# rendeirolab/stainx

Measured on AMD Instinct MI355X. Metric: megapixels/sec Macenko transform, 64x3x512x512 fp32; max-abs vs torch CPU, higher is better.
Workload: dtype f32; 1 GPU; Macenko reference-mode transform, 64x3x512x512 fp32 per GPU (BASELINE configs[1]); tiles_per_gpu=64, height=512, width=512, input_batches_rotated=2, parallelism=tiles sharded over 1 GPU(s), no collective

## Files before the change

stainx_amd/csrc/macenko.hip:

```cpp
#include "common.hpp"

#include <algorithm>
#include <atomic>
#include <type_traits>
#include <cstdlib>

namespace sx {
namespace macenko {

constexpr int kSample = 4096;
constexpr int kMinCap = 8192;
constexpr int kChunk = 16384;
template <typename T> struct PackOf { static constexpr int n = 16 / (int)sizeof(T); };
constexpr int kSlots = 4;
constexpr int kMoments = 20;
constexpr int kPartial = 10;
constexpr int kShortList = 512;
constexpr int kGroupThreads = 1024;
constexpr int kKeys = kSample / kGroupThreads;
constexpr int kPrefetchHist = 8;
constexpr int kPrefetchCand = 8;
static_assert(kKeys * kGroupThreads == kSample && kPrefetchCand * kGroupThreads <= kMinCap, "per-tile stage geometry");

constexpr float kBeta = 0.15f;
// ... 150 lines not shown

constexpr uint32_t kFusedCapMax = 14336;
static bool fused_size(int64_t pixels) { return pixels >= 16384 && pixels <= 262144 && pixels % 4 == 0; }
static uint32_t fused_cap_for(int64_t pixels) { return (uint32_t)std::min<int64_t>(kFusedCapMax, std::max<int64_t>(2048, (pixels / 4 + 255) / 256 * 256)); }
constexpr uint32_t kDenseCapMax = 24576;
static uint32_t dense_cap_for(int64_t pixels) { return (uint32_t)std::min<int64_t>(kDenseCapMax, std::max<int64_t>(2048, (pixels / 8 + 255) / 256 * 256)); }
static uint32_t record_cap_for(int64_t pixels) { return std::max(fused_cap_for(pixels), dense_cap_for(pixels)); }
static size_t dense_spill_words(int64_t pixels) { return dense_cap_for(pixels) > (uint32_t)kLdsKeys ? (size_t)dense_cap_for(pixels) - kLdsKeys : 0; }
constexpr size_t kFusedSchedBytes = 512, kFusedTileBytes = 64;

enum WorkspaceLevel { kWsBase = 0, kWsFused = 1, kWsTwoPass = 2 };
static bool coded_size(int64_t n_tiles, int64_t pixels) { return pixels % 16 == 0 && n_tiles * pixels >= (1ll << 20); }
static size_t coded_bytes(int64_t n_tiles, int64_t pixels) { return align_up(sizeof(uint32_t) * (size_t)n_tiles, 256) + align_up((size_t)3 * pixels * n_tiles, 256); }
static size_t workspace_bytes(int64_t n_tiles, int64_t pixels, int level = kWsTwoPass) {
    const size_t b = (size_t)blocks_per_tile_for(pixels), n = (size_t)n_tiles;
    size_t total = align_up(sizeof(GroupState) * n, 256);
    total += 2 * align_up(sizeof(double) * kPartial * b * n, 256);
    total += align_up(sizeof(uint32_t) * cand_words(n_tiles, pixels), 256);
    total += align_up(sizeof(uint32_t) * 512 * b * n, 256);
    total += align_up(sizeof(float) * 3 * kSample * n, 256);
    total += align_up(sizeof(PoolState), 256);
    if (level >= kWsFused && two_pass_size(pixels)) {
        total += align_up(kPriorRecordBytes * n, 256);
        total += kFusedSchedBytes;
        total += align_up(kFusedTileBytes * n, 256);
        if (fused_size(pixels)) total += align_up(sizeof(uint4) * kSlots * (size_t)record_cap_for(pixels) * n, 256);
        if (fused_size(pixels)) total += align_up(sizeof(uint32_t) * kSlots * dense_spill_words(pixels) * n, 256);
    }
    if (level >= kWsTwoPass && two_pass_size(pixels)) {
        total += align_up(sizeof(float) * 3 * kSlots * (size_t)cap2_for(pixels) * n, 256);
        total += align_up(sizeof(uint32_t) * kSlots * 256 * n, 256);
        total += align_up(sizeof(uint32_t) * kSlots * key_spill_words(pixels) * n, 256);
    }
    return total;
}

static Workspace carve(void* base, int64_t n_tiles, int64_t pixels, size_t codes_at = 0) {
    Workspace w;
    char* p = static_cast<char*>(base);
    const size_t b = (size_t)blocks_per_tile_for(pixels), n = (size_t)n_tiles;
    w.state = reinterpret_cast<GroupState*>(p);
    p += align_up(sizeof(GroupState) * n, 256);
    w.partial = reinterpret_cast<double*>(p);
    p += align_up(sizeof(double) * kPartial * b * n, 256);
    w.partial_all = reinterpret_cast<double*>(p);
    p += align_up(sizeof(double) * kPartial * b * n, 256);
    w.cand = reinterpret_cast<uint32_t*>(p);
    p += align_up(sizeof(uint32_t) * cand_words(n_tiles, pixels), 256);
    w.block_hist = reinterpret_cast<uint32_t*>(p);
    p += align_up(sizeof(uint32_t) * 512 * b * n, 256);
    w.sample_od = reinterpret_cast<float*>(p);
    p += align_up(sizeof(float) * 3 * kSample * n, 256);
    w.pool = reinterpret_cast<PoolState*>(p);
    p += align_up(sizeof(PoolState), 256);
    {
        char* c = codes_at ? static_cast<char*>(base) + codes_at : p;
        w.code_bad = reinterpret_cast<uint32_t*>(c);
        w.codes = reinterpret_cast<uint8_t*>(c + align_up(sizeof(uint32_t) * n, 256));
    }
    w.prior = reinterpret_cast<PriorRecord*>(p);
    p += align_up(kPriorRecordBytes * n, 256);
    w.fsched = reinterpret_cast<FusedSched*>(p);
    p += kFusedSchedBytes;
    w.ftile = reinterpret_cast<FusedTile*>(p);
    p += align_up(kFusedTileBytes * n, 256);
    w.cand_rec = reinterpret_cast<uint4*>(p);
    if (fused_size(pixels)) p += align_up(sizeof(uint4) * kSlots * (size_t)record_cap_for(pixels) * n, 256);
    w.dense_spill = reinterpret_cast<uint32_t*>(p);
    if (fused_size(pixels)) p += align_up(sizeof(uint32_t) * kSlots * dense_spill_words(pixels) * n, 256);
    w.cand_od = reinterpret_cast<float*>(p);
    p += align_up(sizeof(float) * 3 * kSlots * (size_t)cap2_for(pixels) * n, 256);
    w.seg_count = reinterpret_cast<uint32_t*>(p);
    p += align_up(sizeof(uint32_t) * kSlots * 256 * n, 256);
    w.key_spill = reinterpret_cast<uint32_t*>(p);
    return w;
}

template <typename U> __device__ __forceinline__ void put(U* p, U v) { *p = v; }
template <typename U> __device__ __forceinline__ U get(const U* p) { return *p; }

#ifdef SX_STAMPS
#define SX_STAMP(st, i) do { if (threadIdx.x == 0) (st).stamp[i] = (unsigned long long)wall_clock64(); } while (0)
#define SX_UNIT_STAMP(ws, unit, i) do { if (threadIdx.x == 0) reinterpret_cast<unsigned long long*>((ws).block_hist)[(size_t)(unit) * 8 + (i)] = (unsigned long long)wall_clock64(); } while (0)
#else
#define SX_STAMP(st, i) do { } while (0)
#define SX_UNIT_STAMP(ws, unit, i) do { } while (0)
#endif

template <typename T>
__device__ __forceinline__ float log2_level(float raw) {
    const float t = sizeof(T) == 1 ? raw + 1.0f : fmaf(raw, 255.0f, 1.0f);
    return __log2f(t);
}
template <typename T>
__device__ __forceinline__ float optical_density(float raw) {
    return fmaf(-kLn2, log2_level<T>(raw), kLnIo);
}

template <typename T> struct LevelTables {
    __device__ __forceinline__ void fill() {}
};
template <> struct LevelTables<uint8_t> {
    float od[256], l2[256];
    __device__ __forceinline__ void fill() {
        for (int t = threadIdx.x; t < 256; t += blockDim.x) {
            od[t] = optical_density<uint8_t>((float)t);
            l2[t] = log2_level<uint8_t>((float)t);
        }
        __syncthreads();
    }
};
template <typename F> struct Coded {
    uint8_t v;
    __device__ __forceinline__ operator uint32_t() const { return v; }
};
template <typename T> struct Sem { using type = T; };
template <typename F> struct Sem<Coded<F>> { using type = F; };
template <typename F> __device__ __forceinline__ float code_value(int k) {
    return Elem<F>::load(Elem<F>::store(div255_of_level((float)k)));
}
template <typename F> struct LevelTables<Coded<F>> {
    float od[256], l2[256];
    __device__ __forceinline__ void fill() {
        for (int t = threadIdx.x; t < 256; t += blockDim.x) {
            const float v = code_value<F>(t);
            od[t] = optical_density<F>(v);
            l2[t] = log2_level<F>(v);
        }
        __syncthreads();
    }
};
template <typename F, int kCodeCopies> struct CodeTable {
    static constexpr int copies = kCodeCopies;
    uint2 e[256 * kCodeCopies];
    __device__ __forceinline__ void fill() {
        for (int t = threadIdx.x; t < 256; t += blockDim.x) {
            const float v = code_value<F>(t);
            const uint2 entry = make_uint2(__float_as_uint(v), __float_as_uint(optical_density<F>(v)));
#pragma unroll
            for (int c = 0; c < kCodeCopies; ++c) e[t * kCodeCopies + c] = entry;
        }
        __syncthreads();
    }
};
template <typename T, int V, bool kInter> struct Codable { static constexpr bool value = std::is_same<T, float>::value && V == 4 && !kInter; };

template <typename T> __device__ __forceinline__ float od_of(float v, const LevelTables<T>& tb) {
    if constexpr (sizeof(T) == 1) return tb.od[__float_as_uint(v)]; else return optical_density<T>(v);
}
template <typename T> __device__ __forceinline__ float l2_of(float v, const LevelTables<T>& tb) {
    if constexpr (sizeof(T) == 1) return tb.l2[__float_as_uint(v)]; else return log2_level<T>(v);
}

__device__ __forceinline__ bool od_selected(const float od[3], bool use_all) {
    return use_all || (fminf(od[0], fminf(od[1], od[2])) >= kBeta);
}

__device__ __forceinline__ float diamond_angle(float t1, float t0) {
    const float den = fmaxf(fabsf(t0) + fabsf(t1), 1e-30f);
    const float r = t1 * __builtin_amdgcn_rcpf(den);
    return t0 >= 0.0f ? r : (t1 >= 0.0f ? 2.0f - r : -2.0f - r);
}

__device__ __forceinline__ uint32_t angle_key(const float od[3], const float* __restrict__ v) {
    const float t0 = fmaf(od[2], v[4], fmaf(od[1], v[2], od[0] * v[0]));
    const float t1 = fmaf(od[2], v[5], fmaf(od[1], v[3], od[0] * v[1]));
    return float_key(diamond_angle(t1, t0));
}

__device__ inline float angle_from_key(uint32_t key) {
// ... 3134 lines not shown
```

stainx_amd/csrc/macenko_twopass.hpp:

```cpp
#pragma once

namespace sx {
namespace macenko {

constexpr int kPriorSweeps = 4;
constexpr int kPriorUnitsMax = kGroupThreads / 4 * kPriorSweeps;
constexpr int kQueue2 = 512;
constexpr float kSpecSigmasConc = 5.0f, kSpecThresholdScale = 1.0f;
constexpr float kSpecSigmas = 5.0f;
constexpr float kSpecEffFar = 2.0f, kSpecEffNear = 1.0f;
__device__ __forceinline__ float spec_eff(const Geometry& g) { return g.prior_step_q16 >= (8u << 16) ? g.spec_eff_far : g.spec_eff_near; }
constexpr float kSpecKw = 0.10f, kSpecKx = 1.3e-3f;
constexpr float kSpecRot = 0.30f;
constexpr uint32_t kSpecSlow = 1u, kSpecHazard = 2u;
constexpr int kMaxSegments = 256;

constexpr int kRowBelowA = 0, kRowAboveA = 1, kRowBelowB = 2, kRowAboveB = 3, kRowConc = 4, kRowW = 8;
struct alignas(128) PriorRecord {
    float a0[3], a1[3], an[3];
    float rows[16][4];
    float kw, kx;
    float cmax[4];
    int32_t mode;
    int32_t min_first;
// ... 630 lines not shown
                        }
                        if (__builtin_expect(n_q > (uint32_t)(kQueue2 - kWave), 0)) flush();
                    }
                }
                if constexpr (V > 4) __builtin_amdgcn_sched_barrier(0);
            }
            if (++in_run == kShortRun) {
#pragma unroll
                for (int k = 0; k < kPartial; ++k) {
                    acc[k] += (double)m[k];
                    m[k] = 0.0f;
                }
                in_run = 0;
            }
        }
    };
    if (speculate) sweep(std::true_type{}); else sweep(std::false_type{});
    if (in_run) {
#pragma unroll
        for (int k = 0; k < kPartial; ++k) acc[k] += (double)m[k];
    }

    StatsScratch<TPB>* ss = &sh->stats;
#pragma unroll
    for (int k = 0; k < kPartial; ++k) {
        const double s = wave_total_f64(acc[k]);
        if (lane_id() == kWave - 1) ss->red[wave][k] = s;
    }
    if (speculate) {
        flush();
        if (lane_id() == 0) {
            if constexpr (!kFused) {
                uint32_t* counts = ws.seg_count + ((size_t)tile * kSlots) * g.n_seg + seg;
#pragma unroll
                for (int s = 0; s < kSlots; ++s) put(&counts[(size_t)s * g.n_seg], have[s]);
            }
            if (below_a) atomicAdd(&sh->below[0], below_a);
            if (below_b) atomicAdd(&sh->below[1], below_b);
        }
    }
    __syncthreads();
    if (threadIdx.x < kPartial) {
        double s = 0.0;
#pragma unroll
        for (int w = 0; w < TPB / kWave; ++w) s += ss->red[w][threadIdx.x];
        if constexpr (kFused) st_agent(&ws.partial[item * kPartial + threadIdx.x], s); else put(&ws.partial[item * kPartial + threadIdx.x], s);
    }
    if (speculate && threadIdx.x == kPartial) {
        if (sh->below[0]) atomicAdd(&st.below[0], sh->below[0]);
        if (sh->below[1]) atomicAdd(&st.below[1], sh->below[1]);
    }
    double kept_total = 0.0;
#pragma unroll
    for (int w = 0; w < TPB / kWave; ++w) kept_total += ss->red[w][0];
    if (__builtin_expect(kept_total < 3.0, 0)) {
        if (!tile_has_three_kept_witnesses<T, TPB, kInter>(img, g.pixels)) {
            stats_item_all_pixels<T, V, TPB, kInter>(img, g.pixels, p_begin, p_end, ws.partial_all + item * kPartial, ss);
            if constexpr (kFused) __builtin_amdgcn_fence(__ATOMIC_RELEASE, "agent");
        }
    }
    if constexpr (kFused) {
        drain_stores();
        __syncthreads();
        if (threadIdx.x == 0) __hip_atomic_fetch_add(&ws.ftile[tile].a_done, 1u, __ATOMIC_RELAXED, __HIP_MEMORY_SCOPE_AGENT);
    }
}

template <typename T, int V, bool kInter = false, bool kDense = false>
__global__ __launch_bounds__(kStreamThreads, (Codable<T, V, kInter>::value ? 4 : 1)) void pass_a_kernel(const T* __restrict__ images, Geometry g, Workspace ws) {
    __shared__ PassAScratch<kStreamThreads> sh;
    __shared__ LevelTables<T> tb;
    tb.fill();
    if constexpr (Codable<T, V, kInter>::value) {
        if (g.code_epoch != 0u) {
            __shared__ CodeTable<T, 2> ct;
            ct.fill();
            pass_a_item<T, V, kStreamThreads, kInter, kDense, true>(images, g, ws, blockIdx.x / g.blocks_per_tile, blockIdx.x % g.blocks_per_tile, blockIdx.x, &sh, tb, &ct);
            return;
        }
    }
    pass_a_item<T, V, kStreamThreads, kInter, kDense>(images, g, ws, blockIdx.x / g.blocks_per_tile, blockIdx.x % g.blocks_per_tile, blockIdx.x, &sh, tb);
}

struct alignas(16) SlotScratch {
    TileScratch t;
    uint32_t keys[kLdsKeys];
    float vecs[6], pinv[6], he[6];
    double check[8];
    uint32_t lo, hi, n_list, bin, rank_in_bin, result, range_first, range_last, bin_count;
    int ok, use_all;
    unsigned long long n_sel;
    uint32_t seg_prefix[kMaxSegments + 1], seg_total, seg_overflow, over_n;
    uint32_t dense_n;
    uint32_t own_key;
    int partner_ok;
    uint32_t k_floor, k_ceil, n_under;
};

__device__ __forceinline__ void segment_prefix(SlotScratch* sh, const Geometry& g, const Workspace& ws, int tile, int slot) {
    if (threadIdx.x < kWave) {
        const uint32_t* counts = ws.seg_count + ((size_t)tile * kSlots + slot) * g.n_seg;
        uint32_t c[4], sum = 0, raw = 0;
#pragma unroll
        for (int u = 0; u < 4; ++u) {
            const int k = 4 * (int)threadIdx.x + u;
            const uint32_t v = k < g.n_seg ? get(&counts[k]) : 0u;
            raw += v;
            c[u] = min(v, g.seg_cap);
            sum += c[u];
        }
        const uint32_t incl = wave_scan_u32(sum);
        uint32_t run = incl - sum;
#pragma unroll
        for (int u = 0; u < 4; ++u) {
            const int k = 4 * (int)threadIdx.x + u;
            if (k <= g.n_seg) sh->seg_prefix[k] = run;
            run += c[u];
        }
        const uint32_t total_raw = wave_total_u32(raw);
        if (threadIdx.x == kWave - 1) {
            const uint32_t spilled = get(&ws.state[tile].over_count[slot]);
            sh->seg_prefix[g.n_seg] = incl;
            sh->seg_total = total_raw;
            sh->over_n = min(spilled, g.over_cap);
            sh->seg_overflow = spilled > g.over_cap ? 1u : 0u;
        }
    }
}

template <int kPre> struct CandPrefetch {
    float od[kPre][3];
};
template <int kPre>
__device__ __forceinline__ void prefetch_candidates(CandPrefetch<kPre>& pf, const Geometry& g, const float* __restrict__ c0) {
    const uint32_t team = blockDim.x / (uint32_t)g.n_seg, k = threadIdx.x / team, r = threadIdx.x - k * team;
    const float* src = c0 + (size_t)k * g.seg_cap;
#pragma unroll
    for (int u = 0; u < kPre; ++u) {
        const uint32_t o = r + u * team;
        const bool in = k < (uint32_t)g.n_seg && o < g.seg_cap;
#pragma unroll
        for (int c = 0; c < 3; ++c) pf.od[u][c] = in ? get(&src[(size_t)c * g.cap2 + o]) : 0.0f;
    }
}
template <int kPre, class Fn>
__device__ __forceinline__ void for_each_candidate(const CandPrefetch<kPre>& pf, const SlotScratch* sh, const Geometry& g, const float* __restrict__ c0, Fn fn) {
    const uint32_t team = blockDim.x / (uint32_t)g.n_seg, k = threadIdx.x / team, r = threadIdx.x - k * team;
    const bool mine = k < (uint32_t)g.n_seg;
    const uint32_t first = mine ? sh->seg_prefix[k] : 0u, cnt = mine ? sh->seg_prefix[k + 1] - first : 0u;
    const float* src = c0 + (size_t)k * g.seg_cap;
#pragma unroll
    for (int u = 0; u < kPre; ++u) {
        const uint32_t o = r + u * team;
        if (o < cnt) fn(first + o, pf.od[u]);
    }
    constexpr int kFlight = 4;
    for (uint32_t o = threadIdx.x; o < sh->over_n; o += blockDim.x) {
        const float* p = c0 + (size_t)g.n_seg * g.seg_cap + o;
        const float od[3] = {get(&p[0]), get(&p[g.cap2]), get(&p[2 * (size_t)g.cap2])};
        fn(sh->seg_prefix[g.n_seg] + o, od);
    }
    if (k >= (uint32_t)g.n_seg) return;
    for (uint32_t off = r + kPre * team; off < cnt; off += team * kFlight) {
        float od[kFlight][3];
#pragma unroll
        for (int u = 0; u < kFlight; ++u) {
            const uint32_t o = off + u * team;
#pragma unroll
            for (int c = 0; c < 3; ++c) od[u][c] = o < cnt ? get(&src[(size_t)c * g.cap2 + o]) : 0.0f;
        }
#pragma unroll
        for (int u = 0; u < kFlight; ++u) {
            const uint32_t o = off + u * team;
            if (o < cnt) fn(first + o, od[u]);
        }
    }
}

template <int kPre>
__device__ __forceinline__ void prefetch_candidates_dense(CandPrefetch<kPre>& pf, __amdgpu_buffer_rsrc_t rsrc) {
#pragma unroll
    for (int u = 0; u < kPre; ++u) {
        const sx_u4 rec = __builtin_amdgcn_raw_buffer_load_b128(rsrc, (int)((threadIdx.x + (uint32_t)u * blockDim.x) * 16u), 0, 0);
#pragma unroll
        for (int c = 0; c < 3; ++c) pf.od[u][c] = __uint_as_float(rec[c]);
    }
}
template <int kPre, class Fn>
__device__ __forceinline__ void for_each_candidate_dense(const CandPrefetch<kPre>& pf, uint32_t n, __amdgpu_buffer_rsrc_t rsrc, Fn fn) {
#pragma unroll
    for (int u = 0; u < kPre; ++u) {
        const uint32_t i = threadIdx.x + (uint32_t)u * blockDim.x;
        if (i < n) fn(i, pf.od[u]);
    }
    constexpr int kFlight = 4;
    for (uint32_t i0 = threadIdx.x + (uint32_t)kPre * blockDim.x; i0 < n; i0 += blockDim.x * kFlight) {
        float od[kFlight][3];
#pragma unroll
        for (int u = 0; u < kFlight; ++u) {
            const sx_u4 rec = __builtin_amdgcn_raw_buffer_load_b128(rsrc, (int)((i0 + (uint32_t)u * blockDim.x) * 16u), 0, 0);
#pragma unroll
            for (int c = 0; c < 3; ++c) od[u][c] = __uint_as_float(rec[c]);
        }
#pragma unroll
        for (int u = 0; u < kFlight; ++u) {
            const uint32_t i = i0 + (uint32_t)u * blockDim.x;
            if (i < n) fn(i, od[u]);
        }
    }
}
__device__ __forceinline__ void dense_count(SlotScratch* sh, const Geometry& g, const Workspace& ws, int tile, int slot) {
    if (threadIdx.x == kWave - 1) {
        const uint32_t n_raw = get(&ws.ftile[tile].ncand[slot]);
        sh->seg_total = n_raw;
        sh->dense_n = min(n_raw, g.fused_cap);
        sh->over_n = 0;
        sh->seg_overflow = n_raw > g.fused_cap ? 1u : 0u;
    }
}

__device__ __forceinline__ uint32_t slot_key(const SlotScratch* sh, const uint32_t* __restrict__ spill, uint32_t i) { return i < (uint32_t)kLdsKeys ? sh->keys[i] : get(&spill[i - kLdsKeys]); }

__device__ __forceinline__ void select_prepare(SlotScratch* sh) {
    if (threadIdx.x == 0) {
        sh->lo = 0xFFFFFFFFu;
        sh->hi = 0u;
        sh->n_list = 0;
        sh->result = 0;
        sh->n_under = 0;
    }
    for (int i = threadIdx.x; i < 512; i += blockDim.x) (&sh->t.hist_c[0][0])[i] = 0;
}
__device__ __forceinline__ void publish_range(SlotScratch* sh, uint32_t mn, uint32_t mx) {
    mn = wave_min_u32(mn);
    mx = wave_max_u32(mx);
    if (lane_id() == 0 && mn != 0xFFFFFFFFu) {
        atomicMin(&sh->lo, mn);
        atomicMax(&sh->hi, mx);
    }
}

__device__ uint32_t select_slot_keys(SlotScratch* sh, const uint32_t* __restrict__ spill, uint32_t n, uint32_t rank, bool level0_filled, unsigned long long* dbg = nullptr, uint32_t k_floor = 0u, uint32_t k_ceil = 0xFFFFFFFFu) {
    const uint32_t lane = lane_id();
    const int wave = threadIdx.x / kWave;
    const uint32_t share = ((n + blockDim.x - 1) / blockDim.x) | 1u, i_begin = min(threadIdx.x * share, n), i_end = min(i_begin + share, n);
    const uint32_t lo = max(sh->lo, k_floor), hi = max(min(sh->hi, k_ceil), lo);
    double origin = bin_origin_for(lo), scale = bin_scale_for(lo, hi);
    uint32_t k_first = k_floor, k_last = 0xFFFFFFFFu, want = rank;
    uint32_t picked = 0;
    bool by_bin = false;
    uint32_t* hist = sh->t.hist_c[0];
    for (int level = 0; level < 2; ++level) {
        if (level > 0 || !level0_filled) {
            for (uint32_t i = i_begin; i < i_end; ++i) {
                const uint32_t k = slot_key(sh, spill, i);
                if (k >= k_first && k <= k_last) atomicAdd(&hist[bin_of(k, origin, scale)], 1u);
            }
            __syncthreads();
        }
        if (dbg && threadIdx.x == 0) dbg[level] = (unsigned long long)wall_clock64();
        if (wave == 0) {
            uint32_t b, rb;
            scan_pick32(hist, want, b, rb);
            if (lane == 0) {
                const uint32_t in_bin = hist[b];
                sh->bin = b;
                sh->rank_in_bin = rb;
                sh->bin_count = in_bin;
                if (in_bin > (uint32_t)kShortList || level == 1) {
                    uint32_t first, last;
                    bin_key_range(b, origin, scale, first, last);
                    sh->range_first = max(first, k_first);
                    sh->range_last = min(last, k_last);
                }
            }
        }
        __syncthreads();
        want = sh->rank_in_bin;
        picked = sh->bin;
        const uint32_t in_bin = sh->bin_count;
        if (in_bin <= (uint32_t)kShortList && level == 0) {
            by_bin = true;
            break;
        }
        k_first = sh->range_first;
        k_last = sh->range_last;
        if (level == 1) break;
        if (k_first == k_last) return k_first;
        hist = sh->t.hist_c[1];
        origin = bin_origin_for(k_first);
        scale = bin_scale_for(k_first, k_last);
    }
    if (!by_bin && k_first == k_last) return k_first;
    uint32_t* list = &sh->t.keys[0][0];
    for (uint32_t i = i_begin; i < i_end; ++i) {
        const uint32_t k = slot_key(sh, spill, i);
        if (k >= k_first && k <= k_last && (!by_bin || bin_of(k, origin, scale) == picked)) {
            const uint32_t at = atomicAdd(&sh->n_list, 1u);
            if (at < (uint32_t)(2 * kSample)) list[at] = k;
        }
    }
    __syncthreads();
    if (dbg && threadIdx.x == 0) dbg[2] = (unsigned long long)wall_clock64();
    const uint32_t n_list = sh->n_list;
    if (__builtin_expect(n_list <= (uint32_t)kShortList, 1)) {
        rank_pick(list, n_list, want, threadIdx.x, blockDim.x, &sh->result);
        __syncthreads();
        return sh->result;
    }
    if (n_list <= (uint32_t)(2 * kSample)) return radix_select_stream((unsigned long long)n_list, (unsigned long long)want, [list](unsigned long long i, uint32_t& k) { k = list[i]; return true; }, &sh->t);
    return radix_select_stream((unsigned long long)n, (unsigned long long)rank, [sh, spill, k_floor](unsigned long long i, uint32_t& k) { k = slot_key(sh, spill, (uint32_t)i); return k >= k_floor; }, &sh->t);
}

__device__ inline void frame_coordinates(const PriorRecord* pr, const float x[3], float out[3]) {
    const float f00 = pr->a0[0], f10 = pr->a0[1], f20 = pr->a0[2];
    const float f01 = pr->a1[0], f11 = pr->a1[1], f21 = pr->a1[2];
    const float f02 = pr->an[0], f12 = pr->an[1], f22 = pr->an[2];
    const float c00 = f11 * f22 - f12 * f21, c01 = f12 * f20 - f10 * f22, c02 = f10 * f21 - f11 * f20;
    const float det = f00 * c00 + f01 * c01 + f02 * c02;
    const float inv = det != 0.0f ? __builtin_amdgcn_rcpf(det) : 0.0f;
    const float i00 = c00 * inv, i01 = (f02 * f21 - f01 * f22) * inv, i02 = (f01 * f12 - f02 * f11) * inv;
    const float i10 = c01 * inv, i11 = (f00 * f22 - f02 * f20) * inv, i12 = (f02 * f10 - f00 * f12) * inv;
    const float i20 = c02 * inv, i21 = (f01 * f20 - f00 * f21) * inv, i22 = (f00 * f11 - f01 * f10) * inv;
    out[0] = i00 * x[0] + i01 * x[1] + i02 * x[2];
    out[1] = i10 * x[0] + i11 * x[1] + i12 * x[2];
    out[2] = i20 * x[0] + i21 * x[1] + i22 * x[2];
}

template <typename T>
__device__ void exact_plane(const Geometry& g, const Workspace& ws, int tile, SlotScratch* sh) {
    const int64_t first = (int64_t)tile * g.blocks_per_tile;
    if (threadIdx.x < kPartial) {
        double running = 0.0;
        for (int64_t b0 = 0; b0 < g.blocks_per_tile; b0 += 16) {
            double part[16];
#pragma unroll
            for (int u = 0; u < 16; ++u) part[u] = b0 + u < g.blocks_per_tile ? get(&ws.partial[(first + b0 + u) * kPartial + threadIdx.x]) : 0.0;
#pragma unroll
            for (int u = 0; u < 16; ++u)
                if (b0 + u < g.blocks_per_tile) running += part[u];
        }
        sh->t.mom[threadIdx.x] = running;
    }
    if (threadIdx.x == kPartial) sh->t.mom[kPartial] = (double)g.pixels;
    if (threadIdx.x > kPartial && threadIdx.x < kMoments) sh->t.mom[threadIdx.x] = 0.0;
    __syncthreads();
    if (__builtin_expect(sh->t.mom[0] < 3.0, 0)) {
        __syncthreads();
        if (threadIdx.x < kPartial) {
            double running = 0.0;
            for (int64_t b = 0; b < g.blocks_per_tile; ++b) running += get(&ws.partial_all[(first + b) * kPartial + threadIdx.x]);
            sh->t.mom[kPartial + threadIdx.x] = running;
        }
        __syncthreads();
    }
    if (threadIdx.x < 2) {
        double cov[9];
        bool use_all;
        unsigned long long n_sel;
        float vecs[6];
        plane_from_moments<true>(sh->t.mom, true, cov, vecs, use_all, n_sel);
        if (threadIdx.x == 0) {
#pragma unroll
            for (int i = 0; i < 6; ++i) sh->vecs[i] = vecs[i];
            sh->use_all = use_all ? 1 : 0;
            sh->n_sel = n_sel;
            if ((blockIdx.x & 1) == 0) {
                GroupState& st = ws.state[tile];
#pragma unroll
                for (int i = 0; i < 6; ++i) {
                    put(&st.vecs[i], vecs[i]);
                    put(&st.rec[0].coef[i], vecs[i]);
                }
#pragma unroll
                for (int k = 0; k < kMoments; ++k) put(&st.mom[k], sh->t.mom[k]);
#pragma unroll
                for (int i = 0; i < 9; ++i) put(&st.cov[i], cov[i]);
                put(&st.use_all, use_all ? 1 : 0);
                put(&st.rec[0].use_all, use_all ? 1 : 0);
                put(&st.n_sel, n_sel);
            }
        }
    }
    __syncthreads();
}

__device__ inline bool phi_slot_check(const PriorRecord* pr, const float (&v)[6], int j, double (&check)[8], float rot_limit) {
    float m0[3], m1[3];
    const float v0[3] = {v[0], v[2], v[4]}, v1[3] = {v[1], v[3], v[5]};
    frame_coordinates(pr, v0, m0);
    frame_coordinates(pr, v1, m1);
    const float r00 = m0[0], r01 = m0[1], r10 = m1[0], r11 = m1[1], nu0 = m0[2], nu1 = m1[2];
    const float det = r00 * r11 - r01 * r10;
    const float nu = __builtin_amdgcn_sqrtf(nu0 * nu0 + nu1 * nu1);
    const float stretch = __builtin_amdgcn_sqrtf(r00 * r00 + r01 * r01 + r10 * r10 + r11 * r11);
    const float kw = get(&pr->kw), kx = get(&pr->kx);
    bool good = det > 0.9f && stretch < 1.6f && r00 > 0.8f && r11 > 0.8f && fabsf(r01) + fabsf(r10) < rot_limit && kx >= 1.2e-3f;
    {
        const float a1_min = fminf(pr->a1[0], fminf(pr->a1[1], pr->a1[2]));
        const float a0_max = fmaxf(fabsf(pr->a0[0]), fmaxf(fabsf(pr->a0[1]), fabsf(pr->a0[2])));
        const float an_max = fmaxf(fabsf(pr->an[0]), fmaxf(fabsf(pr->an[1]), fabsf(pr->an[2])));
        if (!(r11 * a1_min > 1.05f * (fabsf(r10) * a0_max + nu * an_max))) good = false;
    }
    const uint32_t open = get(&pr->open);
#pragma unroll
    for (int e = 0; e < 2; ++e) {
        const float* row = pr->rows[2 * j + e];
        float gq[3];
        frame_coordinates(pr, row, gq);
        const float dx = gq[1], dy = -gq[0];
        const float mx = r00 * dx + r01 * dy, my = r10 * dx + r11 * dy;
        const bool is_open = ((open >> (2 * j + e)) & 1u) != 0;
        check[e] = is_open ? (e ? 2.0 : 0.0) : (double)diamond_angle(my, mx);
        check[2 + e] = is_open ? 1.0 : 0.0;
        if (!is_open) {
            const float dn = __builtin_amdgcn_sqrtf(dx * dx + dy * dy);
            if (!(my - 0.04f * fabsf(mx) > 0.0f)) good = false;
            if (!(fmaxf(fabsf(row[0]), fmaxf(fabsf(row[1]), fabsf(row[2]))) <= 1.05f)) good = false;
            if (!(nu * stretch * dn * 1.05f <= (kw - fabsf(gq[2])) * det)) good = false;
        }
    }
    if (!(check[1] > check[0])) good = false;
    return good;
}

__device__ inline bool conc_slot_check(const PriorRecord* pr, const float (&pinv)[6], int j, double& theta_out, float& hi_out) {
    const float p[3] = {pinv[3 * j], pinv[3 * j + 1], pinv[3 * j + 2]};
    float gq[3], g1[3], g2[3];
    frame_coordinates(pr, p, gq);
    const float* row1 = pr->rows[kRowConc + 2 * j];
    const float* row2 = pr->rows[kRowConc + 2 * j + 1];
    frame_coordinates(pr, row1, g1);
    frame_coordinates(pr, row2, g2);
    const float u1x = g1[0], u1y = g1[1], t1 = -row1[3], u2x = g2[0], u2y = g2[1], t2 = -row2[3];
    const float det = u1x * u2y - u1y * u2x;
    const float kw = get(&pr->kw), kx = get(&pr->kx);
    if (!(fabsf(det) > 1e-7f)) return false;
    const float inv = __builtin_amdgcn_rcpf(det);
    const float alpha = (gq[0] * u2y - gq[1] * u2x) * inv, beta = (u1x * gq[1] - u1y * gq[0]) * inv;
    const float l1 = fabsf(p[0]) + fabsf(p[1]) + fabsf(p[2]);
    const float rmax = fmaxf(fmaxf(fabsf(row1[0]), fmaxf(fabsf(row1[1]), fabsf(row1[2]))), fmaxf(fabsf(row2[0]), fmaxf(fabsf(row2[1]), fabsf(row2[2]))));
    const bool good = alpha >= 1e-5f * l1 && beta >= 1e-5f * l1 && rmax <= 1.05f && kx >= 1.2e-3f &&
                      (alpha + beta) * kw >= 1.05f * (alpha * fabsf(g1[2]) + beta * fabsf(g2[2]) + fabsf(gq[2])) && (alpha + beta) * (kx - 1.1e-3f) >= 3e-6f * l1 && t1 < 1e30f && t2 < 1e30f;
    theta_out = (double)alpha * (double)t1 + (double)beta * (double)t2;
    const float span = alpha * fmaxf(get(&pr->cmax[2 * j]) - t1, 0.0f) + beta * fmaxf(get(&pr->cmax[2 * j + 1]) - t2, 0.0f);
    hi_out = (float)theta_out + fmaxf(1.25f * span, 1e-3f * fabsf((float)theta_out) + 1e-6f);
    return good;
}

template <typename T, bool kDense = false>
__global__ __launch_bounds__(kGroupThreads) void estimate_stage_kernel(const T* __restrict__ images, Geometry g, Workspace ws, const float* __restrict__ target_max_conc,
                                                                       uint32_t* __restrict__ key_scratch) {
    __shared__ SlotScratch sh;
    const int tile = blockIdx.x >> 1, j = blockIdx.x & 1, slot = 2 + j;
    uint32_t* keep = key_scratch ? key_scratch + ((size_t)tile * 3 + j) * (size_t)g.pixels * (sizeof(T) >= 4 ? sizeof(T) / 4 : 1) : nullptr;
    GroupState& st = ws.state[tile];
    const PriorRecord* pr = &ws.prior[tile];
    const uint32_t below = get(&st.below[j]), spec = get(&st.spec);
    const int mode = get(&pr->mode);
    const bool stamps = j == 0;
    if (stamps) SX_STAMP(st, 8);
    const float* c0 = ws.cand_od + ((size_t)tile * kSlots + j) * 3 * g.cap2;
    const size_t spill_words = kDense ? (g.fused_cap > (uint32_t)kLdsKeys ? g.fused_cap - kLdsKeys : 0u) : (g.cap2 > (uint32_t)kLdsKeys ? g.cap2 - kLdsKeys : 0u);
    uint32_t* const spill_area = kDense ? ws.dense_spill : ws.key_spill;
    const uint4* rec_tile = ws.cand_rec + (size_t)__builtin_amdgcn_readfirstlane(tile) * kSlots * g.fused_cap;
    const auto rsrc_phi = __builtin_amdgcn_make_buffer_rsrc(const_cast<uint4*>(rec_tile + (size_t)__builtin_amdgcn_readfirstlane(j) * g.fused_cap), 0, (int)(g.fused_cap * 16u), 0x00020000);
    const auto rsrc_conc = __builtin_amdgcn_make_buffer_rsrc(const_cast<uint4*>(rec_tile + (size_t)__builtin_amdgcn_readfirstlane(slot) * g.fused_cap), 0, (int)(g.fused_cap * 16u), 0x00020000);
    float v[6];
    bool use_all;
    unsigned long long rank_other;
    {
        CandPrefetch<8> pf;
        if constexpr (kDense) prefetch_candidates_dense(pf, rsrc_phi); else prefetch_candidates(pf, g, c0);
        select_prepare(&sh);
        if constexpr (kDense) dense_count(&sh, g, ws, tile, j); else segment_prefix(&sh, g, ws, tile, j);
        exact_plane<T>(g, ws, tile, &sh);
#pragma unroll
        for (int i = 0; i < 6; ++i) v[i] = sh.vecs[i];
        if (stamps) SX_STAMP(st, 9);
        const uint32_t n = kDense ? sh.dense_n : sh.seg_prefix[g.n_seg] + sh.over_n, n_raw = sh.seg_total;
        use_all = sh.use_all != 0;
        const unsigned long long n_sel = sh.n_sel;
        const unsigned long long rank = nearest_rank_index(j ? 99.0 : 1.0, n_sel);
        rank_other = nearest_rank_index(j ? 1.0 : 99.0, n_sel);
        bool ok = mode == 0 && (spec & (kSpecSlow | kSpecHazard)) == 0 && !use_all && !g.spec_fail && sh.seg_overflow == 0 && rank >= below && rank - below < n;
        uint32_t* spill = spill_area + ((size_t)tile * kSlots + j) * spill_words;
        uint32_t answer = 0, why = 1u;
        if (ok) {
            uint32_t mn = 0xFFFFFFFFu, mx = 0u;
            auto phi_key_of = [&](uint32_t i, const float (&od)[3]) {
                const uint32_t k = angle_key(od, v);
                mn = min(mn, k);
                mx = max(mx, k);
                if (i < (uint32_t)kLdsKeys) sh.keys[i] = k; else put(&spill[i - kLdsKeys], k);
            };
            if constexpr (kDense) for_each_candidate_dense(pf, n, rsrc_phi, phi_key_of); else for_each_candidate(pf, &sh, g, c0, phi_key_of);
            publish_range(&sh, mn, mx);
            if (threadIdx.x == kGroupThreads - 1) sh.ok = phi_slot_check(pr, v, j, sh.check, g.spec_rot) ? 1 : 0;
            __syncthreads();
            if (stamps) SX_STAMP(st, 10);
            ok = sh.ok != 0;
            why = 2u;
        }
        if (ok) {
            answer = select_slot_keys(&sh, spill, n, (uint32_t)(rank - below), false);
            const float a = key_float(answer);
            const double slack = 4e-6;
            if (sh.check[2] == 0.0 && !((double)a >= sh.check[0] + slack)) ok = false;
            if (sh.check[3] == 0.0 && !((double)a <= sh.check[1] - slack)) ok = false;
            why = 3u;
        }
        if (!ok) {
            __syncthreads();
            if (threadIdx.x == 0) {
                atomicOr(&st.fell_back, 1u << j);
                atomicOr(&st.spec, (sh.seg_overflow ? 4u : why) << (8 + 4 * j));
                atomicAdd(&ws.state[0].slow_slots, 1u);
            }
            reset_scratch(&sh.t);
            answer = select_whole_group<T>(images, g, tile, j, rank, v, use_all, &sh.t, keep);
        }
        if (threadIdx.x == 0) {
            put(&st.phi_key[j], answer);
            put(&st.rank[j], rank);
            put(&st.ncand_seen[j], mode == 0 ? n_raw : 0u);
            __hip_atomic_store(&st.phi_pub[j], (1ull << 32) | (unsigned long long)answer, __ATOMIC_RELAXED, __HIP_MEMORY_SCOPE_AGENT);
            sh.own_key = answer;
        }
        if (stamps) SX_STAMP(st, 11);
    }
    if (stamps) SX_STAMP(st, 12);
    const float* c1 = ws.cand_od + ((size_t)tile * kSlots + slot) * 3 * g.cap2;
    CandPrefetch<12> pf;
    if constexpr (kDense) prefetch_candidates_dense(pf, rsrc_conc); else prefetch_candidates(pf, g, c1);
    __syncthreads();
    select_prepare(&sh);
    if constexpr (kDense) dense_count(&sh, g, ws, tile, slot); else segment_prefix(&sh, g, ws, tile, slot);
    auto vectors_and_check = [&](uint32_t partner_key) {
        float he[6], pinv[6];
        const uint32_t key0 = j == 0 ? sh.own_key : partner_key, key1 = j == 0 ? partner_key : sh.own_key;
        stain_vectors_and_pinv(v, key0, key1, he, pinv);
#pragma unroll
        for (int i = 0; i < 6; ++i) {
            sh.pinv[i] = pinv[i];
            sh.he[i] = he[i];
        }
        double theta = 0.0;
        float hi = 0.0f;
        const bool good = mode == 0 && conc_slot_check(pr, pinv, j, theta, hi);
        sh.check[0] = theta;
        sh.ok = good ? 1 : 0;
        const double bound = theta + 4e-6 * fabs(theta) + 1e-7;
        uint32_t kf = float_key((float)bound);
        if ((double)key_float(kf) > bound && kf > 0u) --kf;
        sh.k_floor = good ? kf : 0u;
        sh.k_ceil = good ? max(float_key(hi), kf) : 0xFFFFFFFFu;
    };
    if (threadIdx.x == kWave) {
        unsigned long long granule = 0;
        for (int spin = 0; spin < (1 << 16); ++spin) {
            granule = __hip_atomic_load(&st.phi_pub[1 - j], __ATOMIC_RELAXED, __HIP_MEMORY_SCOPE_AGENT);
            if ((granule >> 32) == 1ull) break;
            __builtin_amdgcn_s_sleep(4);
        }
        sh.partner_ok = (granule >> 32) == 1ull ? 1 : 0;
        if (sh.partner_ok) vectors_and_check((uint32_t)granule);
    }
    __syncthreads();
    if (__builtin_expect(sh.partner_ok == 0, 0)) {
        reset_scratch(&sh.t);
        const uint32_t partner_key = select_whole_group<T>(images, g, tile, 1 - j, rank_other, v, use_all, &sh.t, keep);
        __syncthreads();
        select_prepare(&sh);
        if (threadIdx.x == kWave) vectors_and_check(partner_key);
        __syncthreads();
    }
    float pinv[6];
#pragma unroll
    for (int i = 0; i < 6; ++i) pinv[i] = sh.pinv[i];
    const unsigned long long n_all = (unsigned long long)g.pixels;
    const unsigned long long k99 = nearest_rank_index(99.0, n_all);
    const uint32_t n = kDense ? sh.dense_n : sh.seg_prefix[g.n_seg] + sh.over_n, n_raw = sh.seg_total;
    if (stamps) SX_STAMP(st, 13);
    const unsigned long long outside = n_all - (unsigned long long)n;
    bool ok = mode == 0 && (spec & (kSpecSlow | kSpecHazard)) == 0 && !g.spec_fail && sh.seg_overflow == 0 && k99 >= outside && n > 0;
    uint32_t why = ok && sh.ok == 0 ? 2u : 1u;
    ok = ok && sh.ok != 0;
    uint32_t* spill = spill_area + ((size_t)tile * kSlots + slot) * spill_words;
    uint32_t answer = 0;
    if (ok) {
        const uint32_t k_floor = sh.k_floor, k_ceil = sh.k_ceil;
        uint32_t mn = 0xFFFFFFFFu, mx = 0u, under = 0u;
        auto conc_key_of = [&](uint32_t i, const float (&od)[3]) {
            float ca, cb;
            concentration(od, pinv, ca, cb);
            const uint32_t k = float_key(j ? cb : ca);
            mn = min(mn, k);
            mx = max(mx, k);
            under += k < k_floor ? 1u : 0u;
            if (i < (uint32_t)kLdsKeys) sh.keys[i] = k; else put(&spill[i - kLdsKeys], k);
        };
        if constexpr (kDense) for_each_candidate_dense(pf, n, rsrc_conc, conc_key_of); else for_each_candidate(pf, &sh, g, c1, conc_key_of);
        publish_range(&sh, mn, mx);
        under = wave_total_u32(under);
        if (lane_id() == 0 && under) atomicAdd(&sh.n_under, under);
        __syncthreads();
        if (stamps) SX_STAMP(st, 14);
        const unsigned long long rank_in = k99 - outside;
        const uint32_t n_under = sh.n_under;
        why = 3u;
        if (rank_in < n_under) {
            ok = false;
        } else {
            answer = select_slot_keys(&sh, spill, n, (uint32_t)(rank_in - n_under), false, nullptr, k_floor, k_ceil);
            const double a = (double)key_float(answer), theta = sh.check[0];
            if (!(a >= theta + 4e-6 * fabs(theta) + 1e-7)) ok = false;
        }
    }
    if (!ok) {
        __syncthreads();
        if (threadIdx.x == 0) {
            atomicOr(&st.fell_back, 1u << slot);
            atomicOr(&st.spec, (sh.seg_overflow ? 4u : why) << (8 + 4 * slot));
            atomicAdd(&ws.state[0].slow_slots, 1u);
        }
        reset_scratch(&sh.t);
        answer = select_whole_group<T>(images, g, tile, slot, k99, pinv, true, &sh.t, keep);
    }
    if (threadIdx.x == 0) {
        const float mc = key_float(answer);
        put(&st.max_c[j], mc);
        put(&st.rank[slot], k99);
        put(&st.ncand_seen[slot], mode == 0 ? n_raw : 0u);
        StageRecord* rec = &st.rec[2];
        put(&rec->scale[j], target_max_conc[j] / mc);
        if (j == 0) {
#pragma unroll
            for (int i = 0; i < 6; ++i) {
                put(&rec->coef[i], pinv[i]);
                put(&st.pinv[i], pinv[i]);
                put(&st.he[i], sh.he[i]);
            }
        }
    }
    if (stamps) SX_STAMP(st, 15);
}

}
}
```

Before: 111,400 megapixels/s.

## Hoist global loads to kernel entry and overlap partner polling with prefetch

Moves several global reads in the slot-select kernel (plane partial moments, the prior record, candidate counts) to the start of the kernel so their latency overlaps with the candidate prefetch. The prior record is staged into LDS and the moments are summed from LDS. The wave that polls for the partner's result now issues its prefetch after polling instead of first, so the spin overlaps other waves' loads. Stage timing stamps were also added, but they compile out unless SX_STAMPS is defined. The trade-off is more LDS use (the struct is larger and 128-byte aligned), and the conc buffer resource is now bounded by the raw candidate count.

```diff
diff --git a/stainx_amd/csrc/macenko.hip b/stainx_amd/csrc/macenko.hip
--- a/stainx_amd/csrc/macenko.hip
+++ b/stainx_amd/csrc/macenko.hip
@@ -256,10 +256,20 @@
 #ifdef SX_STAMPS
 #define SX_STAMP(st, i) do { if (threadIdx.x == 0) (st).stamp[i] = (unsigned long long)wall_clock64(); } while (0)
 #define SX_UNIT_STAMP(ws, unit, i) do { if (threadIdx.x == 0) reinterpret_cast<unsigned long long*>((ws).block_hist)[(size_t)(unit) * 8 + (i)] = (unsigned long long)wall_clock64(); } while (0)
+#define SX_STAGE_STAMP_BY(ws, i, t) do { if (threadIdx.x == (t)) reinterpret_cast<unsigned long long*>((ws).block_hist)[(size_t)blockIdx.x * kStageStamps + (i)] = (unsigned long long)wall_clock64(); } while (0)
+#define SX_STAGE_STAMP_CLEAR(ws) do { if (threadIdx.x > 0 && threadIdx.x < kStageStamps) reinterpret_cast<unsigned long long*>((ws).block_hist)[(size_t)blockIdx.x * kStageStamps + threadIdx.x] = 0ull; } while (0)
+#define SX_STAGE_VALUE(ws, i, v) do { if (threadIdx.x == 0) reinterpret_cast<unsigned long long*>((ws).block_hist)[(size_t)blockIdx.x * kStageStamps + (i)] = (unsigned long long)(v); } while (0)
+#define SX_STAGE_STAMP_PTR(ws, i) (reinterpret_cast<unsigned long long*>((ws).block_hist) + (size_t)blockIdx.x * kStageStamps + (i))
 #else
 #define SX_STAMP(st, i) do { } while (0)
 #define SX_UNIT_STAMP(ws, unit, i) do { } while (0)
+#define SX_STAGE_STAMP_BY(ws, i, t) do { } while (0)
+#define SX_STAGE_VALUE(ws, i, v) do { } while (0)
+#define SX_STAGE_STAMP_PTR(ws, i) nullptr
+#define SX_STAGE_STAMP_CLEAR(ws) do { } while (0)
 #endif
+#define SX_STAGE_STAMP(ws, i) SX_STAGE_STAMP_BY(ws, i, 0)
+constexpr int kStageStamps = 32;
 
 template <typename T>
 __device__ __forceinline__ float log2_level(float raw) {
diff --git a/stainx_amd/csrc/macenko_twopass.hpp b/stainx_amd/csrc/macenko_twopass.hpp
--- a/stainx_amd/csrc/macenko_twopass.hpp
+++ b/stainx_amd/csrc/macenko_twopass.hpp
@@ -736,7 +736,7 @@
     pass_a_item<T, V, kStreamThreads, kInter, kDense>(images, g, ws, blockIdx.x / g.blocks_per_tile, blockIdx.x % g.blocks_per_tile, blockIdx.x, &sh, tb);
 }
 
-struct alignas(16) SlotScratch {
+struct alignas(128) SlotScratch {
     TileScratch t;
     uint32_t keys[kLdsKeys];
     float vecs[6], pinv[6], he[6];
@@ -749,6 +749,7 @@
     uint32_t own_key;
     int partner_ok;
     uint32_t k_floor, k_ceil, n_under;
+    PriorRecord prior;
 };
 
 __device__ __forceinline__ void segment_prefix(SlotScratch* sh, const Geometry& g, const Workspace& ws, int tile, int slot) {
@@ -863,9 +864,8 @@
         }
     }
 }
-__device__ __forceinline__ void dense_count(SlotScratch* sh, const Geometry& g, const Workspace& ws, int tile, int slot) {
+__device__ __forceinline__ void dense_count(SlotScratch* sh, const Geometry& g, uint32_t n_raw) {
     if (threadIdx.x == kWave - 1) {
-        const uint32_t n_raw = get(&ws.ftile[tile].ncand[slot]);
         sh->seg_total = n_raw;
         sh->dense_n = min(n_raw, g.fused_cap);
         sh->over_n = 0;
@@ -921,6 +921,7 @@
                 sh->bin = b;
                 sh->rank_in_bin = rb;
                 sh->bin_count = in_bin;
+                if (dbg && level == 0) dbg[3] = in_bin;
                 if (in_bin > (uint32_t)kShortList || level == 1) {
                     uint32_t first, last;
                     bin_key_range(b, origin, scale, first, last);
@@ -955,8 +956,11 @@
         }
     }
     __syncthreads();
-    if (dbg && threadIdx.x == 0) dbg[2] = (unsigned long long)wall_clock64();
     const uint32_t n_list = sh->n_list;
+    if (dbg && threadIdx.x == 0) {
+        dbg[2] = (unsigned long long)wall_clock64();
+        dbg[4] = n_list;
+    }
     if (__builtin_expect(n_list <= (uint32_t)kShortList, 1)) {
         rank_pick(list, n_list, want, threadIdx.x, blockDim.x, &sh->result);
         __syncthreads();
@@ -981,19 +985,22 @@
     out[2] = i20 * x[0] + i21 * x[1] + i22 * x[2];
 }
 
+__device__ __forceinline__ double plane_request(const Geometry& g, const Workspace& ws, int tile) {
+    const uint32_t total = (uint32_t)g.blocks_per_tile * kPartial;
+    return threadIdx.x < total ? get(&ws.partial[(size_t)tile * g.blocks_per_tile * kPartial + threadIdx.x]) : 0.0;
+}
 template <typename T>
-__device__ void exact_plane(const Geometry& g, const Workspace& ws, int tile, SlotScratch* sh) {
+__device__ void exact_plane(const Geometry& g, const Workspace& ws, int tile, SlotScratch* sh, double word) {
     const int64_t first = (int64_t)tile * g.blocks_per_tile;
+    const uint32_t total = (uint32_t)g.blocks_per_tile * kPartial;
+    static_assert(sizeof(sh->t.keys) >= sizeof(double) * 65 * kPartial, "staging room for the work items' moments");
+    double* staged = reinterpret_cast<double*>(&sh->t.keys[0][0]);
+    if (threadIdx.x < total) staged[threadIdx.x] = word;
+    for (uint32_t i = threadIdx.x + blockDim.x; i < total; i += blockDim.x) staged[i] = get(&ws.partial[(size_t)first * kPartial + i]);
+    __syncthreads();
     if (threadIdx.x < kPartial) {
         double running = 0.0;
-        for (int64_t b0 = 0; b0 < g.blocks_per_tile; b0 += 16) {
-            double part[16];
-#pragma unroll
-            for (int u = 0; u < 16; ++u) part[u] = b0 + u < g.blocks_per_tile ? get(&ws.partial[(first + b0 + u) * kPartial + threadIdx.x]) : 0.0;
-#pragma unroll
-            for (int u = 0; u < 16; ++u)
-                if (b0 + u < g.blocks_per_tile) running += part[u];
-        }
+        for (int b = 0; b < g.blocks_per_tile; ++b) running += staged[b * kPartial + threadIdx.x];
         sh->t.mom[threadIdx.x] = running;
     }
     if (threadIdx.x == kPartial) sh->t.mom[kPartial] = (double)g.pixels;
@@ -1109,29 +1116,40 @@
     const int tile = blockIdx.x >> 1, j = blockIdx.x & 1, slot = 2 + j;
     uint32_t* keep = key_scratch ? key_scratch + ((size_t)tile * 3 + j) * (size_t)g.pixels * (sizeof(T) >= 4 ? sizeof(T) / 4 : 1) : nullptr;
     GroupState& st = ws.state[tile];
-    const PriorRecord* pr = &ws.prior[tile];
+    const PriorRecord* pr_global = &ws.prior[tile];
+    const PriorRecord* pr = &sh.prior;
     const uint32_t below = get(&st.below[j]), spec = get(&st.spec);
-    const int mode = get(&pr->mode);
+    const int mode = get(&pr_global->mode);
+    const double plane_word = plane_request(g, ws, tile);
+    constexpr int kPriorWords = (int)(sizeof(PriorRecord) / 4);
+    const uint32_t prior_word = threadIdx.x >= kGroupThreads - kPriorWords ? get(reinterpret_cast<const uint32_t*>(pr_global) + (threadIdx.x - (kGroupThreads - kPriorWords))) : 0u;
+    const uint32_t n_raw_phi = kDense ? get(&ws.ftile[tile].ncand[j]) : 0u, n_raw_conc = kDense ? get(&ws.ftile[tile].ncand[slot]) : 0u;
     const bool stamps = j == 0;
     if (stamps) SX_STAMP(st, 8);
+    SX_STAGE_STAMP(ws, 0);
+    SX_STAGE_STAMP_CLEAR(ws);
     const float* c0 = ws.cand_od + ((size_t)tile * kSlots + j) * 3 * g.cap2;
     const size_t spill_words = kDense ? (g.fused_cap > (uint32_t)kLdsKeys ? g.fused_cap - kLdsKeys : 0u) : (g.cap2 > (uint32_t)kLdsKeys ? g.cap2 - kLdsKeys : 0u);
     uint32_t* const spill_area = kDense ? ws.dense_spill : ws.key_spill;
     const uint4* rec_tile = ws.cand_rec + (size_t)__builtin_amdgcn_readfirstlane(tile) * kSlots * g.fused_cap;
     const auto rsrc_phi = __builtin_amdgcn_make_buffer_rsrc(const_cast<uint4*>(rec_tile + (size_t)__builtin_amdgcn_readfirstlane(j) * g.fused_cap), 0, (int)(g.fused_cap * 16u), 0x00020000);
-    const auto rsrc_conc = __builtin_amdgcn_make_buffer_rsrc(const_cast<uint4*>(rec_tile + (size_t)__builtin_amdgcn_readfirstlane(slot) * g.fused_cap), 0, (int)(g.fused_cap * 16u), 0x00020000);
+    const auto rsrc_conc = __builtin_amdgcn_make_buffer_rsrc(const_cast<uint4*>(rec_tile + (size_t)__builtin_amdgcn_readfirstlane(slot) * g.fused_cap), 0,
+                                                             (int)(min(n_raw_conc, g.fused_cap) * 16u), 0x00020000);
     float v[6];
     bool use_all;
     unsigned long long rank_other;
     {
         CandPrefetch<8> pf;
         if constexpr (kDense) prefetch_candidates_dense(pf, rsrc_phi); else prefetch_candidates(pf, g, c0);
+        SX_STAGE_STAMP(ws, 1);
+        if (threadIdx.x >= kGroupThreads - kPriorWords) reinterpret_cast<uint32_t*>(&sh.prior)[threadIdx.x - (kGroupThreads - kPriorWords)] = prior_word;
         select_prepare(&sh);
-        if constexpr (kDense) dense_count(&sh, g, ws, tile, j); else segment_prefix(&sh, g, ws, tile, j);
-        exact_plane<T>(g, ws, tile, &sh);
+        if constexpr (kDense) dense_count(&sh, g, n_raw_phi); else segment_prefix(&sh, g, ws, tile, j);
+        exact_plane<T>(g, ws, tile, &sh, plane_word);
 #pragma unroll
         for (int i = 0; i < 6; ++i) v[i] = sh.vecs[i];
         if (stamps) SX_STAMP(st, 9);
+        SX_STAGE_STAMP(ws, 2);
         const uint32_t n = kDense ? sh.dense_n : sh.seg_prefix[g.n_seg] + sh.over_n, n_raw = sh.seg_total;
         use_all = sh.use_all != 0;
         const unsigned long long n_sel = sh.n_sel;
@@ -1153,11 +1171,14 @@
             if (threadIdx.x == kGroupThreads - 1) sh.ok = phi_slot_check(pr, v, j, sh.check, g.spec_rot) ? 1 : 0;
             __syncthreads();
             if (stamps) SX_STAMP(st, 10);
+            SX_STAGE_STAMP(ws, 3);
+            SX_STAGE_VALUE(ws, 23, n);
             ok = sh.ok != 0;
             why = 2u;
         }
         if (ok) {
-            answer = select_slot_keys(&sh, spill, n, (uint32_t)(rank - below), false);
+            answer = select_slot_keys(&sh, spill, n, (uint32_t)(rank - below), false, SX_STAGE_STAMP_PTR(ws, 4));
+            SX_STAGE_STAMP(ws, 9);
             const float a = key_float(answer);
             const double slack = 4e-6;
             if (sh.check[2] == 0.0 && !((double)a >= sh.check[0] + slack)) ok = false;
@@ -1182,14 +1203,19 @@
             sh.own_key = answer;
         }
         if (stamps) SX_STAMP(st, 11);
+        SX_STAGE_STAMP(ws, 10);
     }
     if (stamps) SX_STAMP(st, 12);
     const float* c1 = ws.cand_od + ((size_t)tile * kSlots + slot) * 3 * g.cap2;
     CandPrefetch<12> pf;
-    if constexpr (kDense) prefetch_candidates_dense(pf, rsrc_conc); else prefetch_candidates(pf, g, c1);
+    const bool poll_wave = threadIdx.x / kWave == 1;
+    if (!poll_wave) {
+        if constexpr (kDense) prefetch_candidates_dense(pf, rsrc_conc); else prefetch_candidates(pf, g, c1);
+    }
+    SX_STAGE_STAMP(ws, 11);
     __syncthreads();
     select_prepare(&sh);
-    if constexpr (kDense) dense_count(&sh, g, ws, tile, slot); else segment_prefix(&sh, g, ws, tile, slot);
+    if constexpr (kDense) dense_count(&sh, g, n_raw_conc); else segment_prefix(&sh, g, ws, tile, slot);
     auto vectors_and_check = [&](uint32_t partner_key) {
         float he[6], pinv[6];
         const uint32_t key0 = j == 0 ? sh.own_key : partner_key, key1 = j == 0 ? partner_key : sh.own_key;
@@ -1210,15 +1236,21 @@
         sh.k_floor = good ? kf : 0u;
         sh.k_ceil = good ? max(float_key(hi), kf) : 0xFFFFFFFFu;
     };
-    if (threadIdx.x == kWave) {
+    if (poll_wave) {
         unsigned long long granule = 0;
-        for (int spin = 0; spin < (1 << 16); ++spin) {
-            granule = __hip_atomic_load(&st.phi_pub[1 - j], __ATOMIC_RELAXED, __HIP_MEMORY_SCOPE_AGENT);
-            if ((granule >> 32) == 1ull) break;
-            __builtin_amdgcn_s_sleep(4);
-        }
-        sh.partner_ok = (granule >> 32) == 1ull ? 1 : 0;
-        if (sh.partner_ok) vectors_and_check((uint32_t)granule);
+        if (threadIdx.x == kWave) {
+            for (int spin = 0; spin < (1 << 16); ++spin) {
+                granule = __hip_atomic_load(&st.phi_pub[1 - j], __ATOMIC_RELAXED, __HIP_MEMORY_SCOPE_AGENT);
+                if ((granule >> 32) == 1ull) break;
+                __builtin_amdgcn_s_sleep(4);
+            }
+        }
+        if constexpr (kDense) prefetch_candidates_dense(pf, rsrc_conc); else prefetch_candidates(pf, g, c1);
+        if (threadIdx.x == kWave) {
+            sh.partner_ok = (granule >> 32) == 1ull ? 1 : 0;
+            SX_STAGE_STAMP_BY(ws, 12, kWave);
+            if (sh.partner_ok) vectors_and_check((uint32_t)granule);
+        }
     }
     __syncthreads();
     if (__builtin_expect(sh.partner_ok == 0, 0)) {
@@ -1236,6 +1268,7 @@
     const unsigned long long k99 = nearest_rank_index(99.0, n_all);
     const uint32_t n = kDense ? sh.dense_n : sh.seg_prefix[g.n_seg] + sh.over_n, n_raw = sh.seg_total;
     if (stamps) SX_STAMP(st, 13);
+    SX_STAGE_STAMP(ws, 13);
     const unsigned long long outside = n_all - (unsigned long long)n;
     bool ok = mode == 0 && (spec & (kSpecSlow | kSpecHazard)) == 0 && !g.spec_fail && sh.seg_overflow == 0 && k99 >= outside && n > 0;
     uint32_t why = ok && sh.ok == 0 ? 2u : 1u;
@@ -1260,13 +1293,17 @@
         if (lane_id() == 0 && under) atomicAdd(&sh.n_under, under);
         __syncthreads();
         if (stamps) SX_STAMP(st, 14);
+        SX_STAGE_STAMP(ws, 14);
+        SX_STAGE_VALUE(ws, 24, n);
+        SX_STAGE_VALUE(ws, 25, sh.n_under);
         const unsigned long long rank_in = k99 - outside;
         const uint32_t n_under = sh.n_under;
         why = 3u;
         if (rank_in < n_under) {
             ok = false;
         } else {
-            answer = select_slot_keys(&sh, spill, n, (uint32_t)(rank_in - n_under), false, nullptr, k_floor, k_ceil);
+            answer = select_slot_keys(&sh, spill, n, (uint32_t)(rank_in - n_under), false, SX_STAGE_STAMP_PTR(ws, 16), k_floor, k_ceil);
+            SX_STAGE_STAMP(ws, 21);
             const double a = (double)key_float(answer), theta = sh.check[0];
             if (!(a >= theta + 4e-6 * fabs(theta) + 1e-7)) ok = false;
         }
@@ -1298,7 +1335,8 @@
         }
     }
     if (stamps) SX_STAMP(st, 15);
-}
-
-}
-}
+    SX_STAGE_STAMP(ws, 22);
+}
+
+}
+}
```

Measured after the change: 114,700 megapixels/s (median of 6 runs). 3.0% higher.
